# ay-lab/fithic

Measured on AMD Instinct MI355X. Metric: contact-pairs/sec through spline+p-value+BH pass (5 kb cis, whole node), higher is better.
Workload: dtype f64

## Files before the change

fithic_amd/csrc/fhx_bdtrc.hpp:

```cpp
#pragma once
#include <hip/hip_runtime.h>
#include <cstdint>

namespace fhx {
namespace dev {

constexpr double kMachEp = 1.11022302462515654042E-16;
constexpr double kMaxLog = 7.09782712893383996732E2;
constexpr double kMinLog = -7.451332191019412076235E2;
constexpr double kMaxGam = 171.624376956302725;
constexpr double kBig = 4.503599627370496e15;
constexpr double kBigInv = 2.22044604925031308085e-16;

struct BinomTables {
    const double* lbeta;
    const double* inv_beta;
    double n;
    int small_n;
};

__device__ __forceinline__ double cephes_log1p(double x) {
    double z = 1.0 + x;
    if (z < 0.70710678118654752440 || z > 1.41421356237309504880) return log(z);
    z = x * x;
// ... 551 lines not shown
    if (p < 0.0 || p > 1.0 || T.n < fk) return __builtin_nan("");
    if (fk < 0) return 1.0;
    if (fk == T.n) return 0.0;
    const double dn = T.n - fk;
    if (count == 1) {
        if (p < 0.01) return -cephes_expm1(dn * cephes_log1p(-p));
        return 1.0 - pow(1.0 - p, dn);
    }
    return incbet(fk + 1.0, dn, p, T.lbeta[count], T.small_n ? T.inv_beta[count] : 0.0);
}

__device__ __forceinline__ double bdtrc_count_trivial(int count, const BinomTables& T, double p) {
    if (isnan(p)) return p;
    const double fk = (double)count - 1.0;
    if (p < 0.0 || p > 1.0 || T.n < fk) return __builtin_nan("");
    if (fk < 0) return 1.0;
    if (fk == T.n) return 0.0;
    const double dn = T.n - fk;
    if (count == 1) {
        if (p < 0.01) return -cephes_expm1(dn * cephes_log1p(-p));
        return 1.0 - pow(1.0 - p, dn);
    }
    return p <= 0.0 ? 0.0 : 1.0;
}

__device__ __forceinline__ bool bdtrc_is_closed_form(int count, double n_total, double p) {
    return count == 1 && p >= 0.0 && p <= 1.0 && n_total > 0.0;
}
__device__ __forceinline__ double bdtrc_closed_form(double n_total, double p) {
    if (p < 0.01) return -cephes_expm1(n_total * cephes_log1p(-p));
    return 1.0 - pow(1.0 - p, n_total);
}

__device__ __forceinline__ double bdtrc_count_trivial_open(int count, const BinomTables& T, double p) {
    if (isnan(p)) return p;
    const double fk = (double)count - 1.0;
    if (p < 0.0 || p > 1.0 || T.n < fk) return __builtin_nan("");
    if (fk < 0) return 1.0;
    if (fk == T.n) return 0.0;
    return p <= 0.0 ? 0.0 : 1.0;
}

__device__ __forceinline__ int bdtrc_class(int count, double n_total, double p) {
    if (isnan(p)) return BC_TRIVIAL;
    const double fk = (double)count - 1.0;
    if (p < 0.0 || p > 1.0 || n_total < fk || fk < 0 || fk == n_total || count == 1) return BC_TRIVIAL;
    const double aa = fk + 1.0, bb = n_total - fk, xx = p;
    if (xx <= 0.0 || xx >= 1.0) return BC_TRIVIAL;
    if (bb * xx <= 1.0 && xx <= 0.95) return BC_PSERIES;
    const double w = 1.0 - xx;
    double a, b, x;
    bool swapped;
    if (xx > aa / (aa + bb)) {
        swapped = true; a = bb; b = aa; x = w;
        if (b * x <= 1.0 && x <= 0.95) return BC_PSERIES;
    } else {
        swapped = false; a = aa; b = bb; x = xx;
    }
    const double y = x * (a + b - 2.0) - (a - 1.0);
    if (y < 0.0) return swapped ? BC_CF_SWAPPED : BC_CF_BCF;
    return BC_CF_BD;
}

struct ClsRow {
    double tA, tB, tC, tD, tE, pad0, pad1, pad2;
};

__device__ __forceinline__ bool cls_pred(int which, double aa, double bb, double xx) {
    const double w = 1.0 - xx;
    switch (which) {
        case 0: return bb * xx <= 1.0 && xx <= 0.95;
        case 2: return aa * w <= 1.0 && w <= 0.95;
// ... 116 lines not shown
```

fithic_amd/csrc/fhx_ctx.hpp:

```cpp
#pragma once
#include <hip/hip_runtime.h>

#include <atomic>
#include <functional>
#include <chrono>
#include <thread>
#include <memory>
#include <sys/stat.h>
#include <unistd.h>
#include <deque>
#include <mutex>
#include <map>
#include <condition_variable>
#include <algorithm>
#include <climits>
#include <cstddef>
#include <cmath>
#include <cstdio>
#include <cstdlib>
#include <cstring>
#include <string>
#include <vector>

#include "../../include/fithic_mi355x.h"
// ... 61 lines not shown
    int n_table;
    double min_x, max_x;
    long long dist_low, dist_up;
    double total_intra, total_inter;
};

constexpr int K2_THREADS = 256;

constexpr int K2_QUEUES = dev::BC_COUNT - 1;

struct QEntry {
    unsigned int row;
    int count;
    double prior;
};

constexpr int K2_MAX_SHARDS = 2048;

struct QSpan {
    QEntry* base;
    long long cap_s;
    int dir;
    int n_shards;
    const unsigned long long* count;
};
__device__ __forceinline__ QEntry* qentry(const QSpan& q, int shard, long long j) {
    return q.base + (long long)shard * q.cap_s + (long long)q.dir * j;
}

struct K2Queues {
    QSpan q[K2_QUEUES + 1];
    unsigned long long* count;
    unsigned int* heavy_hist;
};

constexpr int K2H_BUCKETS = 2048;
constexpr int K2H_BLOCKS = 1024;
__device__ __forceinline__ int k2h_bucket(int signed_count);

struct CutoffToHost {
    volatile unsigned long long* words = nullptr;
    unsigned long long ticket = 0;
    unsigned int* done = nullptr;
    unsigned long long* zero_me = nullptr;
};

constexpr int K3_DENSE_PERCENT = 35;
constexpr int K2_COUNTER_WORDS = 8;
constexpr int FDR_BUCKETS = 51;

struct DeviceWords {
    unsigned long long bh_kept;
    unsigned long long bh_cutoff;
    unsigned long long bh_below;
    unsigned long long array_kept;
    unsigned long long array_cutoff;
    unsigned long long sort_n;
    unsigned long long run_total;
    unsigned long long nf_keys;
    unsigned long long outliers_added;
    unsigned long long first_dup;
    unsigned long long memo_overflow;
    alignas(128) unsigned long long k2_redo;
    unsigned long long k2_next[K2_COUNTER_WORDS - 1];
    alignas(128) unsigned long long k3_dense;
    unsigned long long k3_sparse;
// ... 343 lines not shown
    DeviceScratch() = default;
    explicit DeviceScratch(ScratchPool* p) : pool(p) {}
    ~DeviceScratch() {
        for (auto& b : v) {
            if (pool)
                pool->give(b.first, b.second);
            else
                (void)hipFree(b.first);
        }
    }
    template <typename T>
    hipError_t get(T** p, size_t bytes) {
        bytes = std::max<size_t>(bytes, 16);
        if (pool) {
            size_t real = 0;
            if (void* q = pool->take(bytes, &real)) {
                *p = (T*)q;
                v.emplace_back(q, real);
                return hipSuccess;
            }
        }
        const hipError_t e = hipMalloc((void**)p, bytes);
        if (e == hipSuccess) v.emplace_back((void*)*p, bytes);
        return e;
    }
};

inline int grid_for(int64_t n, int threads, int max_blocks = 256 * 8) {
    const int64_t b = (n + threads - 1) / threads;
    return (int)std::max<int64_t>(1, std::min<int64_t>(b, max_blocks));
}

inline int k2_classify_grid(int64_t n) {
    return grid_for(n, K2_CL_TILE, K2_MAX_SHARDS);
}
inline long long k2_shard_capacity(int64_t n) {
    const long long tiles = std::max<long long>(1, (n + K2_CL_TILE - 1) / K2_CL_TILE), grid = k2_classify_grid(n);
    return ((tiles + grid - 1) / grid) * (long long)K2_CL_TILE;
}


int build_slot_tables(fhx_ctx* ctx);
int run_ids(fhx_ctx* ctx, const unsigned long long* keys, int64_t n, unsigned int* ids, unsigned int* tile_scratch, int64_t* n_runs);
int alloc_row_arrays(fhx_ctx* ctx, int64_t n, int64_t n_dist);
int ingest_device_rows_nonfixed(fhx_ctx* ctx, const int32_t* c1, const int32_t* m1, const int32_t* c2, const int32_t* m2,
                                const int32_t* cnt, int64_t n);
int ingest_device_rows(fhx_ctx* ctx, const int32_t* c1, const int32_t* m1, const int32_t* c2, const int32_t* m2, const int32_t* cnt,
                       int64_t n);
int pass_stats_nonfixed(fhx_ctx* ctx, fhx_stats* out);
int launch_k1(fhx_ctx* ctx);
void fold_kernel_events(fhx_ctx* ctx);
void before_rerecord(fhx_ctx* ctx, int group);
K2Params make_k2_params(fhx_ctx* c);
void launch_k2_extras(fhx_ctx* ctx, const K2Params& P, int64_t n_rows, double* d_expcc, double* d_b1, double* d_b2);
int ensure_sort_scratch(fhx_ctx* ctx);
int sort_blocks_for(int64_t n_hint);
int radix_sort_pairs(fhx_ctx* ctx, unsigned long long* keys[2], unsigned int* vals[2], const unsigned long long* counter, int passes,
                     int* result_buf, int64_t n_hint = -1);
void launch_rs_scan(fhx_ctx* ctx, int nblk);
int fill_top_hist(fhx_ctx* ctx);
void launch_k3_cutoff(fhx_ctx* ctx, const unsigned long long* hist, double n_tests, unsigned long long* d_cutoff,
                      unsigned long long* n_below, unsigned long long dense_min, unsigned long long* dense_flag, const CutoffToHost& host,
                      unsigned long long sparse_max = 0, unsigned long long* sparse_flag = nullptr);
void launch_bh_tile_max(fhx_ctx* ctx, int tiles, const unsigned long long* keys, const unsigned long long* n_ptr, int64_t n_fixed,
                        double n_tests, double rank0, double* tile_max);
void launch_bh_scan_tiles(fhx_ctx* ctx, double* tile_max, const unsigned long long* n_ptr, int64_t n_fixed, double carry_in,
// ... 10 lines not shown
```

fithic_amd/csrc/fhx_k2.hip:

```cpp
#include "fhx_ctx.hpp"

namespace fhx {

__device__ __forceinline__ double prior_by_search(const K2Params& P, long long dist) {
    double look = (double)dist;
    if (look < P.min_x) look = P.min_x;
    if (look > P.max_x) look = P.max_x;
    int lo = 0, hi = P.n_table;
    while (lo < hi) {
        const int mid = (lo + hi) >> 1;
        if (P.table_x[mid] < look)
            lo = mid + 1;
        else
            hi = mid;
    }
    return P.table_y[min(lo, P.n_table - 1)];
}

template <int NF = -1>
__device__ __forceinline__ bool row_prior(const K2Params& P, int l1, int l2, double& prior, bool& is_inter) {
    const bool inter = l2 < 0;
    const int s2 = inter ? ~l2 : l2;
    const double b1 = P.no_bias ? 1.0 : P.slot_bias[l1], b2 = P.no_bias ? 1.0 : P.slot_bias[s2];
    if ((b1 < 0 || b2 < 0) && !inter) return false;
    if (!inter && P.mode != FHX_MODE_INTER_ONLY) {
        if (NF == 1 || (NF == -1 && P.nonfixed)) {
            const long long dist = llabs((long long)P.slot_mid[l1] - (long long)P.slot_mid[s2]);
            if (dist < P.dist_low || dist > P.dist_up) return false;
            prior = prior_by_search(P, dist) * (b1 * b2);
            is_inter = false;
            return true;
        }
        const int d = abs(l1 - s2);
        if (d < P.lo_idx || d > P.hi_idx) return false;
        prior = P.prior_lut[d] * (b1 * b2);
        is_inter = false;
        return true;
    }
    if (P.mode == FHX_MODE_INTRA_ONLY) return false;
    prior = P.inter_chr_prob * (b1 * b2);
    is_inter = true;
    return true;
}

template <int ITEMS>
__device__ __forceinline__ void rows_prior_fixed(const K2Params& P, const int (&l1)[ITEMS], const int (&l2)[ITEMS], double (&prior)[ITEMS],
                                                 bool (&is_inter)[ITEMS], bool (&live)[ITEMS]) {
    double b1[ITEMS], b2[ITEMS], tab[ITEMS];
    int dist[ITEMS];
#pragma unroll
    for (int r = 0; r < ITEMS; ++r) {
        const bool inter = l2[r] < 0;
        const int s2 = inter ? ~l2[r] : l2[r];
        dist[r] = abs(l1[r] - s2);
        b1[r] = P.no_bias ? 1.0 : P.slot_bias[l1[r]];
        b2[r] = P.no_bias ? 1.0 : P.slot_bias[s2];
        tab[r] = P.prior_lut[min(dist[r], P.lut_len - 1)];
    }
#pragma unroll
    for (int r = 0; r < ITEMS; ++r) {
        const bool inter = l2[r] < 0;
        const double bb = b1[r] * b2[r];
        const bool as_intra = !inter && P.mode != FHX_MODE_INTER_ONLY;
        const bool discarded = (b1[r] < 0 || b2[r] < 0) && !inter;
        const bool in_range = dist[r] >= P.lo_idx && dist[r] <= P.hi_idx;
        live[r] = !discarded && (as_intra ? in_range : P.mode != FHX_MODE_INTRA_ONLY);
        is_inter[r] = !as_intra;
        prior[r] = live[r] ? (as_intra ? tab[r] : P.inter_chr_prob) * bb : 1.0;
    }
}

constexpr int K2_HIST_BINS = 4096;
struct FusedHist {
    unsigned int* h;
    unsigned int ones;
    bool on;
    __device__ __forceinline__ void init(unsigned int* lds, const unsigned long long* global) {
        h = lds;
        ones = 0;
        on = global != nullptr;
        if (on) {
            for (int i = threadIdx.x; i < K2_HIST_BINS; i += blockDim.x) h[i] = 0;
            __syncthreads();
        }
    }
    __device__ __forceinline__ void add(double v) {
        if (!on) return;
        if (v == 1.0)
            ++ones;
        else if (v == v) {
            unsigned long long bits = (unsigned long long)__double_as_longlong(v);
            if (bits == 0x8000000000000000ull) bits = 0ull;
            atomicAdd(&h[min((unsigned int)(bits >> 50), (unsigned int)K2_HIST_BINS - 1u)], 1u);
        }
    }
    __device__ __forceinline__ void add_wave_min(double v, bool valid) {
        if (!on) return;
        valid = valid && v == v;
        unsigned long long key = valid ? (unsigned long long)__double_as_longlong(v) : ~0ull;
        if (key == 0x8000000000000000ull) key = 0ull;
#pragma unroll
        for (int s = 32; s >= 1; s >>= 1) {
            const unsigned long long o = __shfl_xor(key, s, 64);
            key = o < key ? o : key;
        }
        const unsigned int n = (unsigned int)__popcll(__ballot(valid));
        if ((threadIdx.x & 63) == 0 && n) atomicAdd(&h[min((unsigned int)(key >> 50), (unsigned int)K2_HIST_BINS - 1u)], n);
    }
    __device__ __forceinline__ void flush(unsigned long long* global) {
        if (!on) return;
        const unsigned int w = (unsigned int)wave_sum_i64((long long)ones);
        if ((threadIdx.x & 63) == 0 && w) atomicAdd(&h[0x3FF0000000000000ull >> 50], w);
        __syncthreads();
        for (int i = threadIdx.x; i < K2_HIST_BINS; i += blockDim.x)
            if (h[i]) atomicAdd(&global[i], (unsigned long long)h[i]);
    }
};

template <bool SCATTERED>
__device__ __forceinline__ void store_p(double* dst, double v) {
    if (SCATTERED)
        __builtin_nontemporal_store(v, dst);
    else
        *dst = v;
}

constexpr int K2_TB_COUNTS = 128;
template <int NF, int WPE, int TABLE, bool HOIST = false, bool PACK = false>
__global__ __launch_bounds__(K2_THREADS) __attribute__((amdgpu_waves_per_eu(WPE, WPE))) void k2_classify(K2Params P, K2Queues Q) {
    static_assert(!HOIST || NF == 0, "the hoisted gathers are the fixed-size path's");
    static_assert(TABLE == 0 || TABLE == 3, "table variants 1 and 2 were measured and dropped");
    constexpr int ITEMS = K2_CL_ITEMS, WAVES = K2_THREADS / 64, WAVE_ROWS = 64 * ITEMS;
    __shared__ unsigned int cnt[K2_QUEUES + 1];
    __shared__ double cf_prior[WAVES][WAVE_ROWS];
    __shared__ unsigned short cf_idx[WAVES][WAVE_ROWS];
    __shared__ unsigned int hist_lds[K2_HIST_BINS];
    __shared__ unsigned int heavy_lds[K2H_BUCKETS];
    __shared__ double tb_lds[TABLE == 3 ? 2 * K2_TB_COUNTS : 1];
    if (TABLE == 3) {
        static_assert(2 * K2_TB_COUNTS <= K2_THREADS, "one thread per table entry");
        if (threadIdx.x < 2 * K2_TB_COUNTS) {
            const int c = threadIdx.x & (K2_TB_COUNTS - 1);
            const double n_total = threadIdx.x < K2_TB_COUNTS ? P.intra.n : P.inter.n;
            const double fk = (double)c - 1.0;
            const double aa = fk + 1.0, bb = n_total - fk;
            tb_lds[threadIdx.x] = aa / (aa + bb);
        }
    }
    if (threadIdx.x <= K2_QUEUES) cnt[threadIdx.x] = 0;
    const bool count_heavy = Q.heavy_hist != nullptr;
    if (count_heavy)
        for (int d = threadIdx.x; d < K2H_BUCKETS; d += K2_THREADS) heavy_lds[d] = 0;
    FusedHist H;
    H.init(hist_lds, P.top_hist);
    __syncthreads();
    const int lane = threadIdx.x & 63;
    const int wave = threadIdx.x >> 6;
    const unsigned long long lane_lt = (1ull << lane) - 1ull;
    const int shard = (int)blockIdx.x;
    const int64_t tiles = (P.n + K2_CL_TILE - 1) / K2_CL_TILE;
    const int4* a4 = reinterpret_cast<const int4*>(P.loc1);
    const int4* b4 = reinterpret_cast<const int4*>(P.loc2);
    const int4* c4 = reinterpret_cast<const int4*>(P.count);
    for (int64_t t = blockIdx.x; t < tiles; t += gridDim.x) {
        const int64_t wave_row0 = t * K2_CL_TILE + (int64_t)wave * WAVE_ROWS;
        const int64_t row0 = wave_row0 + lane * ITEMS;
        int l1_of[ITEMS] = {0, 0, 0, 0}, l2_of[ITEMS] = {0, 0, 0, 0}, count_of[ITEMS] = {0, 0, 0, 0};
        if (row0 < P.n) {
            const int4 a = a4[row0 >> 2], b = b4[row0 >> 2], c = c4[row0 >> 2];
            l1_of[0] = a.x; l1_of[1] = a.y; l1_of[2] = a.z; l1_of[3] = a.w;
            l2_of[0] = b.x; l2_of[1] = b.y; l2_of[2] = b.z; l2_of[3] = b.w;
            count_of[0] = c.x; count_of[1] = c.y; count_of[2] = c.z; count_of[3] = c.w;
            if (HOIST && row0 + ITEMS > P.n) {
#pragma unroll
                for (int r = 1; r < ITEMS; ++r)
                    if (row0 + r >= P.n) l1_of[r] = l2_of[r] = 0;
            }
        }
        int cls_of[ITEMS];
        double prior_of[ITEMS];
        bool inter_of[ITEMS], live_of[ITEMS];
        if (HOIST) rows_prior_fixed<ITEMS>(P, l1_of, l2_of, prior_of, inter_of, live_of);
#pragma unroll
        for (int r = 0; r < ITEMS; ++r) {
            const int64_t i = row0 + r;
            int cls = -1;
            double prior = 1.0;
            int c = count_of[r];
            if (i < P.n) {
                double pv = 1.0;
                bool is_inter = false;
                cls = 0;
                bool live;
                if (HOIST) {
                    live = live_of[r];
                    prior = prior_of[r];
                    is_inter = inter_of[r];
                } else {
                    live = row_prior<NF>(P, l1_of[r], l2_of[r], prior, is_inter);
                }
                if (live) {
                    const dev::BinomTables& T = is_inter ? P.inter : P.intra;
                    if (TABLE == 3) {
                        double tB;
                        if (c >= 0 && c < K2_TB_COUNTS) {
                            tB = tb_lds[(is_inter ? K2_TB_COUNTS : 0) + c];
                        } else {
                            const double fk = (double)c - 1.0;
                            const double aa = fk + 1.0, bb = T.n - fk;
                            tB = aa / (aa + bb);
                        }
                        cls = dev::bdtrc_class_tb(c, T.n, prior, tB);
                    } else {
                        cls = dev::bdtrc_class(c, T.n, prior);
                    }
                    if (cls == dev::BC_TRIVIAL) {
                        if (dev::bdtrc_is_closed_form(c, T.n, prior))
                            cls = prior < 0.01 ? K2_CLOSED_LOCAL : K2_CLOSED;
                        else
                            pv = dev::bdtrc_count_trivial_open(c, T, prior);
                    }
                    if (is_inter) c = -c;
                }
                if (cls == 0) {
                    P.p[i] = pv;
                    H.add(pv);
                }
            }
            cls_of[r] = cls;
            count_of[r] = c;
            prior_of[r] = prior;
        }
        unsigned int before_cls[ITEMS];
        unsigned int tot[K2_CLASSES] = {0u, 0u, 0u, 0u, 0u, 0u};
        static_assert(K2_CLASSES == 6 && K2_QUEUES == 4, "lane k reserves class k; the sixth class is wave-local");
        if (PACK) {
            unsigned int mine[2] = {0u, 0u};
            unsigned int shift_of[ITEMS];
#pragma unroll
            for (int r = 0; r < ITEMS; ++r) {
                const int k = cls_of[r] - 1;
                const int f = k >= 3 ? k - 3 : k;
                shift_of[r] = 10u * (unsigned int)(f < 0 ? 0 : f);
                const unsigned int one = k >= 0 ? (1u << shift_of[r]) : 0u;
                mine[0] += k < 3 ? one : 0u;
                mine[1] += k >= 3 ? one : 0u;
            }
            const unsigned int incl0 = wave_incl_sum_u32(mine[0]), incl1 = wave_incl_sum_u32(mine[1]);
            const unsigned int all0 = (unsigned int)__builtin_amdgcn_readlane((int)incl0, 63), all1 = (unsigned int)__builtin_amdgcn_readlane((int)incl1, 63);
            tot[0] = all0 & 1023u; tot[1] = (all0 >> 10) & 1023u; tot[2] = (all0 >> 20) & 1023u;
            tot[3] = all1 & 1023u; tot[4] = (all1 >> 10) & 1023u; tot[5] = (all1 >> 20) & 1023u;
            unsigned int run[2] = {incl0 - mine[0], incl1 - mine[1]};
#pragma unroll
            for (int r = 0; r < ITEMS; ++r) {
                const int k = cls_of[r] - 1;
                const unsigned int word = k >= 3 ? run[1] : run[0];
                before_cls[r] = (word >> shift_of[r]) & 1023u;
                const unsigned int one = k >= 0 ? (1u << shift_of[r]) : 0u;
                run[0] += k < 3 ? one : 0u;
                run[1] += k >= 3 ? one : 0u;
            }
        } else {
#pragma unroll
            for (int r = 0; r < ITEMS; ++r) {
                before_cls[r] = 0;
#pragma unroll
                for (int k = 1; k <= K2_CLASSES; ++k) {
                    const unsigned long long m = __ballot(cls_of[r] == k);
                    if (cls_of[r] == k) before_cls[r] = tot[k - 1] + (unsigned int)__popcll(m & lane_lt);
                    tot[k - 1] += (unsigned int)__popcll(m);
                }
            }
        }
        const unsigned int my_tot = lane == 0 ? tot[0] : (lane == 1 ? tot[1] : (lane == 2 ? tot[2] : (lane == 3 ? tot[3] : tot[4])));
        unsigned int my_base = 0;
        if (lane <= K2_QUEUES && my_tot) my_base = atomicAdd(&cnt[lane], my_tot);
        unsigned int wave_base[K2_QUEUES + 1];
#pragma unroll
        for (int k = 0; k <= K2_QUEUES; ++k) wave_base[k] = __shfl(my_base, k, 64);
#pragma unroll
        for (int r = 0; r < ITEMS; ++r) {
            const int k = cls_of[r] - 1;
            if (k >= 0 && k <= K2_QUEUES) {
                const unsigned int wb = k == 0 ? wave_base[0] : (k == 1 ? wave_base[1] : (k == 2 ? wave_base[2] : (k == 3 ? wave_base[3] : wave_base[4])));
                QEntry e;
                e.row = (unsigned int)(row0 + r);
                e.count = count_of[r];
                e.prior = prior_of[r];
                *qentry(Q.q[k], shard, (long long)(wb + before_cls[r])) = e;
                if (k == dev::BC_CF_SWAPPED - 1 && count_heavy) atomicAdd(&heavy_lds[k2h_bucket(e.count)], 1u);
            } else if (cls_of[r] == K2_CLOSED_LOCAL) {
                cf_prior[wave][before_cls[r]] = prior_of[r];
                cf_idx[wave][before_cls[r]] = (unsigned short)((lane * ITEMS + r) | (count_of[r] < 0 ? 0x8000 : 0));
            }
        }
        __builtin_amdgcn_fence(__ATOMIC_RELEASE, "wavefront");
        __builtin_amdgcn_wave_barrier();
        __builtin_amdgcn_fence(__ATOMIC_ACQUIRE, "wavefront");
        const unsigned int n_local = tot[K2_CLASSES - 1];
        for (unsigned int j = lane; j < n_local; j += 64) {
            const unsigned int ix = cf_idx[wave][j];
            const double n_total = (ix & 0x8000u) ? P.inter.n : P.intra.n;
            const double pr = cf_prior[wave][j];
            const double pv = -dev::cephes_expm1(n_total * dev::cephes_log1p(-pr));
            P.p[wave_row0 + (ix & 0x7FFFu)] = pv;
            H.add(pv);
        }
        __builtin_amdgcn_fence(__ATOMIC_RELEASE, "wavefront");
        __builtin_amdgcn_wave_barrier();
    }
    __syncthreads();
    if (threadIdx.x <= K2_QUEUES) Q.count[(size_t)threadIdx.x * K2_MAX_SHARDS + shard] = cnt[threadIdx.x];
    if (count_heavy)
        for (int d = threadIdx.x; d < K2H_BUCKETS; d += K2_THREADS)
            if (heavy_lds[d]) atomicAdd(&Q.heavy_hist[(size_t)d * K2H_BLOCKS + (shard & (K2H_BLOCKS - 1))], heavy_lds[d]);
    H.flush(P.top_hist);
}

__global__ __launch_bounds__(K2_THREADS) void k2_closed(K2Params P, QSpan q, unsigned long long* __restrict__ zero_words,
                                                        unsigned long long* __restrict__ cutoff_word) {
    __shared__ unsigned int hist_lds[K2_HIST_BINS];
    if (blockIdx.x == 0 && threadIdx.x < K2_COUNTER_WORDS) zero_words[threadIdx.x] = 0ull;
    if (blockIdx.x == 0 && threadIdx.x == K2_COUNTER_WORDS) *cutoff_word = KEY_KEEP_ALL;
    FusedHist H;
    H.init(hist_lds, P.top_hist);
    for (int sh = blockIdx.x; sh < q.n_shards; sh += gridDim.x) {
        const long long n = (long long)q.count[sh];
        for (long long j = threadIdx.x; j < n; j += blockDim.x) {
            const QEntry e = *qentry(q, sh, j);
            const double pv = dev::bdtrc_closed_form(e.count < 0 ? P.inter.n : P.intra.n, e.prior);
            store_p<false>(P.p + e.row, pv);
            H.add(pv);
        }
    }
    H.flush(P.top_hist);
}

struct QDense {
    static constexpr int PAIRS = K2_MAX_SHARDS / 2;
    unsigned int* prefix;
    const unsigned long long* count;
    __device__ __forceinline__ void build(const QSpan& q, unsigned int* prefix_lds, unsigned int* wave_tot) {
        static_assert(PAIRS % K2_THREADS == 0, "whole pairs per thread");
        constexpr int PER = PAIRS / K2_THREADS;
        prefix = prefix_lds;
        count = q.count;
        unsigned int c[PER], s = 0;
#pragma unroll
// ... 628 lines not shown
    if (Q->heavy_hist && !prezeroed)
        FHX_HIP(hipMemsetAsync(ctx->d_block_hist, 0, (size_t)K2H_BUCKETS * K2H_BLOCKS * sizeof(unsigned int), ctx->stream));
    ctx->k2_shards = plan.n_shards;
    auto span = [&](int cls, QEntry* buf, int dir) {
        Q->q[cls - 1] = QSpan{dir > 0 ? buf : buf + plan.cap_s - 1, plan.cap_s, dir, plan.n_shards, Q->count + (size_t)(cls - 1) * K2_MAX_SHARDS};
    };
    span(dev::BC_CF_SWAPPED, ctx->d_queue[0], 1);
    span(dev::BC_PSERIES, ctx->d_queue[0], -1);
    span(dev::BC_CF_BCF, ctx->d_queue[1], 1);
    span(dev::BC_CF_BD, ctx->d_queue[1], -1);
    span(K2_CLOSED, ctx->d_queue_sorted, 1);
    return FHX_OK;
}

template <int CLS, bool SMALL_N>
static void launch_k2_queue(fhx_ctx* ctx, const K2Params& P, const K2Queues& Q) {
    hipLaunchKernelGGL(HIP_KERNEL_NAME(k2_queue<CLS, SMALL_N>), dim3(2 * resident_grid(ctx, k2_queue<CLS, SMALL_N>)), dim3(K2_THREADS), 0,
                       ctx->stream, P, Q.q[CLS - 1]);
}
template <int CLS, bool SMALL_N>
static void launch_k2_queue_by_count(fhx_ctx* ctx, const K2Params& P, const K2Queues& Q) {
    constexpr int PIECE = SMALL_N ? 4 : 5;
    hipLaunchKernelGGL(HIP_KERNEL_NAME(k2_queue_by_count<CLS, SMALL_N, PIECE>), dim3(resident_grid(ctx, k2_queue_by_count<CLS, SMALL_N, PIECE>)),
                       dim3(K2_THREADS), 0, ctx->stream, P, Q.q[CLS - 1], (unsigned int*)(ctx->d_words->k2_next + CLS));
}
template <int ROWS, int WAVES, bool SMALL_N>
static void launch_k2h_heavy(fhx_ctx* ctx, const K2Params& P, QEntry* redo) {
    hipLaunchKernelGGL(HIP_KERNEL_NAME(k2h_heavy<ROWS, WAVES, SMALL_N>), dim3(256 * WAVES), dim3(K2H_THREADS), 0, ctx->stream,
                       K2HeavyParams{P.intra, P.inter, P.p, P.top_hist}, (const QEntry*)ctx->d_queue_sorted, (const unsigned int*)ctx->d_k2h_off,
                       (const unsigned int*)ctx->d_digit_total, (const dev::CfRow*)ctx->d_cf_tab, redo, &ctx->d_words->k2_redo,
                       (unsigned int*)ctx->d_words->k2_next);
}

template <bool SMALL_N>
static int launch_k2(fhx_ctx* ctx, const K2Plan& plan, const K2Params& P, const K2Queues& Q) {
    const dim3 cgrid(plan.n_shards), block(K2_THREADS);
    if (P.nonfixed)
        hipLaunchKernelGGL(HIP_KERNEL_NAME(k2_classify<1, 4, 0>), cgrid, block, 0, ctx->stream, P, Q);
    else
        hipLaunchKernelGGL(HIP_KERNEL_NAME(k2_classify<0, 4, 3, true, true>), cgrid, block, 0, ctx->stream, P, Q);
    hipLaunchKernelGGL(k2_closed, dim3(256 * 8), block, 0, ctx->stream, P, Q.q[K2_CLOSED - 1], &ctx->d_words->k2_redo, &ctx->d_words->bh_cutoff);
    if (plan.legacy_heavy) {
        FHX_HIP(hipEventRecord(ctx->ev[6], ctx->stream));
        launch_k2_queue<dev::BC_CF_SWAPPED, SMALL_N>(ctx, P, Q);
        FHX_HIP(hipEventRecord(ctx->ev[7], ctx->stream));
        ctx->ev_folded[3] = false;
        launch_k2_queue_by_count<dev::BC_CF_BD, SMALL_N>(ctx, P, Q);
        launch_k2_queue_by_count<dev::BC_CF_BCF, SMALL_N>(ctx, P, Q);
        launch_k2_queue<dev::BC_PSERIES, SMALL_N>(ctx, P, Q);
        return FHX_OK;
    }
    static_assert(K2H_BUCKETS == RADIX && K2H_BLOCKS == SORT_BLOCKS, "the radix sort's count matrix and scan are reused");
    QEntry* hq = ctx->d_queue[0];
    launch_rs_scan(ctx, (int)SORT_BLOCKS);
    hipLaunchKernelGGL(k2h_offsets_and_tables, dim3(K2H_GENERIC + 1), dim3(1024), 0, ctx->stream, (const unsigned int*)ctx->d_digit_total,
                       ctx->d_k2h_off, 64u * (unsigned int)plan.heavy_rows, P.intra.n, P.inter.n, ctx->d_cf_tab);
    hipLaunchKernelGGL(k2h_scatter, dim3(K2H_BLOCKS), dim3(K2H_THREADS), 0, ctx->stream, Q.q[dev::BC_CF_SWAPPED - 1],
                       (const unsigned int*)ctx->d_block_hist, (const unsigned int*)ctx->d_k2h_off, ctx->d_queue_sorted);
    launch_k2_queue<dev::BC_PSERIES, SMALL_N>(ctx, P, Q);
    FHX_HIP(hipEventRecord(ctx->ev[6], ctx->stream));
    if (plan.heavy_rows == 2) launch_k2h_heavy<2, 8, SMALL_N>(ctx, P, hq);
    else launch_k2h_heavy<4, 4, SMALL_N>(ctx, P, hq);
    FHX_HIP(hipEventRecord(ctx->ev[7], ctx->stream));
    ctx->ev_folded[3] = false;
    hipLaunchKernelGGL(k2h_generic, dim3(256 * 4), dim3(K2_THREADS), 0, ctx->stream, P, (const QEntry*)ctx->d_queue_sorted,
                       (const unsigned int*)ctx->d_k2h_off, (const unsigned int*)ctx->d_digit_total, (const QEntry*)hq,
                       (const unsigned long long*)&ctx->d_words->k2_redo);
    launch_k2_queue_by_count<dev::BC_CF_BD, SMALL_N>(ctx, P, Q);
    launch_k2_queue_by_count<dev::BC_CF_BCF, SMALL_N>(ctx, P, Q);
    return FHX_OK;
}

static int k2_fused_hist(fhx_ctx* ctx, bool prezeroed, K2Params* P) {
// ... 480 lines not shown
```

Before: 14.17 billion.

## Slim k2_classify kernel arguments and specialize on no_bias

Replaces the large K2Params/K2Queues kernel arguments of the classify kernel with a compact dedicated parameter struct that flattens queue bases, directions and mode flags. It adds a compile-time no_bias specialization and computes per-wave queue pointers once through LDS instead of shuffling bases. It also restructures the per-row loop so that dead rows are written up front and the packed prefix-count path is always used. The aim is to cut scalar argument loads, VALU work and register pressure in the classify pass, at the cost of more template variants and an added env override for grid size.

```diff
diff --git a/fithic_amd/csrc/fhx_bdtrc.hpp b/fithic_amd/csrc/fhx_bdtrc.hpp
--- a/fithic_amd/csrc/fhx_bdtrc.hpp
+++ b/fithic_amd/csrc/fhx_bdtrc.hpp
@@ -607,12 +607,12 @@
     return 1.0 - pow(1.0 - p, n_total);
 }
 
-__device__ __forceinline__ double bdtrc_count_trivial_open(int count, const BinomTables& T, double p) {
+__device__ __forceinline__ double bdtrc_count_trivial_open(int count, double n_total, double p) {
     if (isnan(p)) return p;
     const double fk = (double)count - 1.0;
-    if (p < 0.0 || p > 1.0 || T.n < fk) return __builtin_nan("");
+    if (p < 0.0 || p > 1.0 || n_total < fk) return __builtin_nan("");
     if (fk < 0) return 1.0;
-    if (fk == T.n) return 0.0;
+    if (fk == n_total) return 0.0;
     return p <= 0.0 ? 0.0 : 1.0;
 }
 
diff --git a/fithic_amd/csrc/fhx_ctx.hpp b/fithic_amd/csrc/fhx_ctx.hpp
--- a/fithic_amd/csrc/fhx_ctx.hpp
+++ b/fithic_amd/csrc/fhx_ctx.hpp
@@ -117,6 +117,33 @@
     QSpan q[K2_QUEUES + 1];
     unsigned long long* count;
     unsigned int* heavy_hist;
+};
+
+struct K2ClassifyParams {
+    const int32_t *loc1, *loc2, *count;
+    const double* slot_bias;
+    const double* prior_lut;
+    double* p;
+    unsigned long long* top_hist;
+    QEntry* q_base[K2_QUEUES + 1];
+    unsigned long long* q_count;
+    unsigned int* heavy_hist;
+    long long cap_s;
+    int64_t n;
+    double n_intra, n_inter;
+    double inter_chr_prob;
+    int lut_len, lo_idx, hi_idx;
+    unsigned int q_down;
+    bool intra_by_distance;
+    bool other_rows_live;
+};
+struct K2ClassifyParamsNF : K2ClassifyParams {
+    const int32_t* slot_mid;
+    const double *table_x, *table_y;
+    int n_table, mode;
+    double min_x, max_x;
+    long long dist_low, dist_up;
+    bool no_bias;
 };
 
 constexpr int K2H_BUCKETS = 2048;
@@ -526,6 +553,10 @@
 }
 
 inline int k2_classify_grid(int64_t n) {
+    if (const char* e = std::getenv("FHX_K2_CLASSIFY_GRID")) {
+        const long long g = std::atoll(e);
+        if (g >= 1) return (int)std::min<long long>(g, K2_MAX_SHARDS);
+    }
     return grid_for(n, K2_CL_TILE, K2_MAX_SHARDS);
 }
 inline long long k2_shard_capacity(int64_t n) {
diff --git a/fithic_amd/csrc/fhx_k2.hip b/fithic_amd/csrc/fhx_k2.hip
--- a/fithic_amd/csrc/fhx_k2.hip
+++ b/fithic_amd/csrc/fhx_k2.hip
@@ -2,7 +2,8 @@
 
 namespace fhx {
 
-__device__ __forceinline__ double prior_by_search(const K2Params& P, long long dist) {
+template <class PT>
+__device__ __forceinline__ double prior_by_search(const PT& P, long long dist) {
     double look = (double)dist;
     if (look < P.min_x) look = P.min_x;
     if (look > P.max_x) look = P.max_x;
@@ -17,14 +18,16 @@
     return P.table_y[min(lo, P.n_table - 1)];
 }
 
-template <int NF = -1>
-__device__ __forceinline__ bool row_prior(const K2Params& P, int l1, int l2, double& prior, bool& is_inter) {
+template <int NF = -1, class PT = K2Params>
+__device__ __forceinline__ bool row_prior(const PT& P, int l1, int l2, double& prior, bool& is_inter) {
     const bool inter = l2 < 0;
     const int s2 = inter ? ~l2 : l2;
     const double b1 = P.no_bias ? 1.0 : P.slot_bias[l1], b2 = P.no_bias ? 1.0 : P.slot_bias[s2];
     if ((b1 < 0 || b2 < 0) && !inter) return false;
     if (!inter && P.mode != FHX_MODE_INTER_ONLY) {
-        if (NF == 1 || (NF == -1 && P.nonfixed)) {
+        bool by_search = NF == 1;
+        if constexpr (NF == -1) by_search = P.nonfixed;
+        if (by_search) {
             const long long dist = llabs((long long)P.slot_mid[l1] - (long long)P.slot_mid[s2]);
             if (dist < P.dist_low || dist > P.dist_up) return false;
             prior = prior_by_search(P, dist) * (b1 * b2);
@@ -43,9 +46,9 @@
     return true;
 }
 
-template <int ITEMS>
-__device__ __forceinline__ void rows_prior_fixed(const K2Params& P, const int (&l1)[ITEMS], const int (&l2)[ITEMS], double (&prior)[ITEMS],
-                                                 bool (&is_inter)[ITEMS], bool (&live)[ITEMS]) {
+template <int ITEMS, bool NO_BIAS>
+__device__ __forceinline__ void rows_prior_fixed(const K2ClassifyParams& P, const int (&l1)[ITEMS], const int (&l2)[ITEMS],
+                                                 double (&prior)[ITEMS], bool (&is_inter)[ITEMS], bool (&live)[ITEMS]) {
     double b1[ITEMS], b2[ITEMS], tab[ITEMS];
     int dist[ITEMS];
 #pragma unroll
@@ -53,18 +56,18 @@
         const bool inter = l2[r] < 0;
         const int s2 = inter ? ~l2[r] : l2[r];
         dist[r] = abs(l1[r] - s2);
-        b1[r] = P.no_bias ? 1.0 : P.slot_bias[l1[r]];
-        b2[r] = P.no_bias ? 1.0 : P.slot_bias[s2];
+        b1[r] = NO_BIAS ? 1.0 : P.slot_bias[l1[r]];
+        b2[r] = NO_BIAS ? 1.0 : P.slot_bias[s2];
         tab[r] = P.prior_lut[min(dist[r], P.lut_len - 1)];
     }
 #pragma unroll
     for (int r = 0; r < ITEMS; ++r) {
         const bool inter = l2[r] < 0;
         const double bb = b1[r] * b2[r];
-        const bool as_intra = !inter && P.mode != FHX_MODE_INTER_ONLY;
+        const bool as_intra = !inter && P.intra_by_distance;
         const bool discarded = (b1[r] < 0 || b2[r] < 0) && !inter;
         const bool in_range = dist[r] >= P.lo_idx && dist[r] <= P.hi_idx;
-        live[r] = !discarded && (as_intra ? in_range : P.mode != FHX_MODE_INTRA_ONLY);
+        live[r] = live[r] && !discarded && (as_intra ? in_range : P.other_rows_live);
         is_inter[r] = !as_intra;
         prior[r] = live[r] ? (as_intra ? tab[r] : P.inter_chr_prob) * bb : 1.0;
     }
@@ -126,29 +129,36 @@
 }
 
 constexpr int K2_TB_COUNTS = 128;
-template <int NF, int WPE, int TABLE, bool HOIST = false, bool PACK = false>
-__global__ __launch_bounds__(K2_THREADS) __attribute__((amdgpu_waves_per_eu(WPE, WPE))) void k2_classify(K2Params P, K2Queues Q) {
-    static_assert(!HOIST || NF == 0, "the hoisted gathers are the fixed-size path's");
-    static_assert(TABLE == 0 || TABLE == 3, "table variants 1 and 2 were measured and dropped");
+template <int NF>
+struct K2ClassifyArgs {
+    using type = K2ClassifyParams;
+};
+template <>
+struct K2ClassifyArgs<1> {
+    using type = K2ClassifyParamsNF;
+};
+template <int NF, bool NO_BIAS>
+__global__ __launch_bounds__(K2_THREADS) __attribute__((amdgpu_waves_per_eu(4, 4))) void k2_classify(const typename K2ClassifyArgs<NF>::type P) {
+    static_assert(NF == 0 || NF == 1, "fixed-size loci or arbitrary ones");
+    static_assert(NF == 0 || !NO_BIAS, "k2_classify<1> reads no_bias at run time (row_prior<1>)");
     constexpr int ITEMS = K2_CL_ITEMS, WAVES = K2_THREADS / 64, WAVE_ROWS = 64 * ITEMS;
     __shared__ unsigned int cnt[K2_QUEUES + 1];
+    __shared__ QEntry* wave_q[WAVES][8];
     __shared__ double cf_prior[WAVES][WAVE_ROWS];
     __shared__ unsigned short cf_idx[WAVES][WAVE_ROWS];
     __shared__ unsigned int hist_lds[K2_HIST_BINS];
     __shared__ unsigned int heavy_lds[K2H_BUCKETS];
-    __shared__ double tb_lds[TABLE == 3 ? 2 * K2_TB_COUNTS : 1];
-    if (TABLE == 3) {
-        static_assert(2 * K2_TB_COUNTS <= K2_THREADS, "one thread per table entry");
-        if (threadIdx.x < 2 * K2_TB_COUNTS) {
-            const int c = threadIdx.x & (K2_TB_COUNTS - 1);
-            const double n_total = threadIdx.x < K2_TB_COUNTS ? P.intra.n : P.inter.n;
-            const double fk = (double)c - 1.0;
-            const double aa = fk + 1.0, bb = n_total - fk;
-            tb_lds[threadIdx.x] = aa / (aa + bb);
-        }
+    __shared__ double tb_lds[2 * K2_TB_COUNTS];
+    static_assert(2 * K2_TB_COUNTS <= K2_THREADS, "one thread per table entry");
+    if (threadIdx.x < 2 * K2_TB_COUNTS) {
+        const int c = threadIdx.x & (K2_TB_COUNTS - 1);
+        const double n_total = threadIdx.x < K2_TB_COUNTS ? P.n_intra : P.n_inter;
+        const double fk = (double)c - 1.0;
+        const double aa = fk + 1.0, bb = n_total - fk;
+        tb_lds[threadIdx.x] = aa / (aa + bb);
     }
     if (threadIdx.x <= K2_QUEUES) cnt[threadIdx.x] = 0;
-    const bool count_heavy = Q.heavy_hist != nullptr;
+    const bool count_heavy = P.heavy_hist != nullptr;
     if (count_heavy)
         for (int d = threadIdx.x; d < K2H_BUCKETS; d += K2_THREADS) heavy_lds[d] = 0;
     FusedHist H;
@@ -156,8 +166,19 @@
     __syncthreads();
     const int lane = threadIdx.x & 63;
     const int wave = threadIdx.x >> 6;
-    const unsigned long long lane_lt = (1ull << lane) - 1ull;
     const int shard = (int)blockIdx.x;
+    static_assert(K2_QUEUES + 1 == 5, "five queues: lanes 0..4");
+    QEntry* my_q = nullptr;
+    {
+        const long long region = (long long)shard * P.cap_s;
+        QEntry* const q0 = P.q_base[0];
+        QEntry* const q1 = P.q_base[1];
+        QEntry* const q2 = P.q_base[2];
+        QEntry* const q3 = P.q_base[3];
+        QEntry* const q4 = P.q_base[4];
+        my_q = (lane == 0 ? q0 : (lane == 1 ? q1 : (lane == 2 ? q2 : (lane == 3 ? q3 : q4)))) + region;
+    }
+    const bool my_down = ((P.q_down >> (lane & 7)) & 1u) != 0u;
     const int64_t tiles = (P.n + K2_CL_TILE - 1) / K2_CL_TILE;
     const int4* a4 = reinterpret_cast<const int4*>(P.loc1);
     const int4* b4 = reinterpret_cast<const int4*>(P.loc2);
@@ -165,142 +186,128 @@
     for (int64_t t = blockIdx.x; t < tiles; t += gridDim.x) {
         const int64_t wave_row0 = t * K2_CL_TILE + (int64_t)wave * WAVE_ROWS;
         const int64_t row0 = wave_row0 + lane * ITEMS;
+        const int64_t left = P.n - row0;
+        const int n_here = left >= ITEMS ? ITEMS : (left > 0 ? (int)left : 0);
         int l1_of[ITEMS] = {0, 0, 0, 0}, l2_of[ITEMS] = {0, 0, 0, 0}, count_of[ITEMS] = {0, 0, 0, 0};
-        if (row0 < P.n) {
+        if (n_here > 0) {
             const int4 a = a4[row0 >> 2], b = b4[row0 >> 2], c = c4[row0 >> 2];
             l1_of[0] = a.x; l1_of[1] = a.y; l1_of[2] = a.z; l1_of[3] = a.w;
             l2_of[0] = b.x; l2_of[1] = b.y; l2_of[2] = b.z; l2_of[3] = b.w;
             count_of[0] = c.x; count_of[1] = c.y; count_of[2] = c.z; count_of[3] = c.w;
-            if (HOIST && row0 + ITEMS > P.n) {
+            if (NF == 0 && n_here < ITEMS) {
 #pragma unroll
                 for (int r = 1; r < ITEMS; ++r)
-                    if (row0 + r >= P.n) l1_of[r] = l2_of[r] = 0;
+                    if (r >= n_here) l1_of[r] = l2_of[r] = 0;
             }
         }
-        int cls_of[ITEMS];
         double prior_of[ITEMS];
         bool inter_of[ITEMS], live_of[ITEMS];
-        if (HOIST) rows_prior_fixed<ITEMS>(P, l1_of, l2_of, prior_of, inter_of, live_of);
+#pragma unroll
+        for (int r = 0; r < ITEMS; ++r) live_of[r] = r < n_here;
+        if constexpr (NF == 0) {
+            rows_prior_fixed<ITEMS, NO_BIAS>(P, l1_of, l2_of, prior_of, inter_of, live_of);
+        } else {
+#pragma unroll
+            for (int r = 0; r < ITEMS; ++r) {
+                prior_of[r] = 1.0;
+                inter_of[r] = false;
+                if (live_of[r]) live_of[r] = row_prior<NF>(P, l1_of[r], l2_of[r], prior_of[r], inter_of[r]);
+            }
+        }
+        double* const p_lane = P.p + row0;
 #pragma unroll
         for (int r = 0; r < ITEMS; ++r) {
-            const int64_t i = row0 + r;
+            if (r < n_here && !live_of[r]) {
+                p_lane[r] = 1.0;
+                ++H.ones;
+            }
+        }
+        int cls_of[ITEMS];
+#pragma unroll
+        for (int r = 0; r < ITEMS; ++r) {
             int cls = -1;
-            double prior = 1.0;
-            int c = count_of[r];
-            if (i < P.n) {
-                double pv = 1.0;
-                bool is_inter = false;
-                cls = 0;
-                bool live;
-                if (HOIST) {
-                    live = live_of[r];
-                    prior = prior_of[r];
-                    is_inter = inter_of[r];
+            if (live_of[r]) {
+                const int c = count_of[r];
+                const double n_total = inter_of[r] ? P.n_inter : P.n_intra;
+                double tB;
+                if (c >= 0 && c < K2_TB_COUNTS) {
+                    tB = tb_lds[(inter_of[r] ? K2_TB_COUNTS : 0) + c];
                 } else {
-                    live = row_prior<NF>(P, l1_of[r], l2_of[r], prior, is_inter);
+                    const double fk = (double)c - 1.0;
+                    const double aa = fk + 1.0, bb = n_total - fk;
+                    tB = aa / (aa + bb);
                 }
-                if (live) {
-                    const dev::BinomTables& T = is_inter ? P.inter : P.intra;
-                    if (TABLE == 3) {
-                        double tB;
-                        if (c >= 0 && c < K2_TB_COUNTS) {
-                            tB = tb_lds[(is_inter ? K2_TB_COUNTS : 0) + c];
-                        } else {
-                            const double fk = (double)c - 1.0;
-                            const double aa = fk + 1.0, bb = T.n - fk;
-                            tB = aa / (aa + bb);
-                        }
-                        cls = dev::bdtrc_class_tb(c, T.n, prior, tB);
+                cls = dev::bdtrc_class_tb(c, n_total, prior_of[r], tB);
+                if (cls == dev::BC_TRIVIAL) {
+                    if (dev::bdtrc_is_closed_form(c, n_total, prior_of[r])) {
+                        cls = prior_of[r] < 0.01 ? K2_CLOSED_LOCAL : K2_CLOSED;
                     } else {
-                        cls = dev::bdtrc_class(c, T.n, prior);
+                        const double pv = dev::bdtrc_count_trivial_open(c, n_total, prior_of[r]);
+                        p_lane[r] = pv;
+                        H.add(pv);
+                        cls = -1;
                     }
-                    if (cls == dev::BC_TRIVIAL) {
-                        if (dev::bdtrc_is_closed_form(c, T.n, prior))
-                            cls = prior < 0.01 ? K2_CLOSED_LOCAL : K2_CLOSED;
-                        else
-                            pv = dev::bdtrc_count_trivial_open(c, T, prior);
-                    }
-                    if (is_inter) c = -c;
-                }
-                if (cls == 0) {
-                    P.p[i] = pv;
-                    H.add(pv);
                 }
             }
             cls_of[r] = cls;
-            count_of[r] = c;
-            prior_of[r] = prior;
         }
         unsigned int before_cls[ITEMS];
-        unsigned int tot[K2_CLASSES] = {0u, 0u, 0u, 0u, 0u, 0u};
         static_assert(K2_CLASSES == 6 && K2_QUEUES == 4, "lane k reserves class k; the sixth class is wave-local");
-        if (PACK) {
-            unsigned int mine[2] = {0u, 0u};
-            unsigned int shift_of[ITEMS];
-#pragma unroll
-            for (int r = 0; r < ITEMS; ++r) {
-                const int k = cls_of[r] - 1;
-                const int f = k >= 3 ? k - 3 : k;
-                shift_of[r] = 10u * (unsigned int)(f < 0 ? 0 : f);
-                const unsigned int one = k >= 0 ? (1u << shift_of[r]) : 0u;
-                mine[0] += k < 3 ? one : 0u;
-                mine[1] += k >= 3 ? one : 0u;
-            }
-            const unsigned int incl0 = wave_incl_sum_u32(mine[0]), incl1 = wave_incl_sum_u32(mine[1]);
-            const unsigned int all0 = (unsigned int)__builtin_amdgcn_readlane((int)incl0, 63), all1 = (unsigned int)__builtin_amdgcn_readlane((int)incl1, 63);
-            tot[0] = all0 & 1023u; tot[1] = (all0 >> 10) & 1023u; tot[2] = (all0 >> 20) & 1023u;
-            tot[3] = all1 & 1023u; tot[4] = (all1 >> 10) & 1023u; tot[5] = (all1 >> 20) & 1023u;
-            unsigned int run[2] = {incl0 - mine[0], incl1 - mine[1]};
-#pragma unroll
-            for (int r = 0; r < ITEMS; ++r) {
-                const int k = cls_of[r] - 1;
-                const unsigned int word = k >= 3 ? run[1] : run[0];
-                before_cls[r] = (word >> shift_of[r]) & 1023u;
-                const unsigned int one = k >= 0 ? (1u << shift_of[r]) : 0u;
-                run[0] += k < 3 ? one : 0u;
-                run[1] += k >= 3 ? one : 0u;
-            }
-        } else {
-#pragma unroll
-            for (int r = 0; r < ITEMS; ++r) {
-                before_cls[r] = 0;
-#pragma unroll
-                for (int k = 1; k <= K2_CLASSES; ++k) {
-                    const unsigned long long m = __ballot(cls_of[r] == k);
-                    if (cls_of[r] == k) before_cls[r] = tot[k - 1] + (unsigned int)__popcll(m & lane_lt);
-                    tot[k - 1] += (unsigned int)__popcll(m);
-                }
-            }
-        }
-        const unsigned int my_tot = lane == 0 ? tot[0] : (lane == 1 ? tot[1] : (lane == 2 ? tot[2] : (lane == 3 ? tot[3] : tot[4])));
-        unsigned int my_base = 0;
-        if (lane <= K2_QUEUES && my_tot) my_base = atomicAdd(&cnt[lane], my_tot);
-        unsigned int wave_base[K2_QUEUES + 1];
-#pragma unroll
-        for (int k = 0; k <= K2_QUEUES; ++k) wave_base[k] = __shfl(my_base, k, 64);
+        unsigned int mine[2] = {0u, 0u};
+        unsigned int shift_of[ITEMS];
+#pragma unroll
+        for (int r = 0; r < ITEMS; ++r) {
+            const int k = cls_of[r] - 1;
+            const int f = k >= 3 ? k - 3 : k;
+            shift_of[r] = 10u * (unsigned int)(f < 0 ? 0 : f);
+            const unsigned int one = k >= 0 ? (1u << shift_of[r]) : 0u;
+            mine[0] += k < 3 ? one : 0u;
+            mine[1] += k >= 3 ? one : 0u;
+        }
+        const unsigned int incl0 = wave_incl_sum_u32(mine[0]), incl1 = wave_incl_sum_u32(mine[1]);
+        const unsigned int all0 = (unsigned int)__builtin_amdgcn_readlane((int)incl0, 63), all1 = (unsigned int)__builtin_amdgcn_readlane((int)incl1, 63);
+        unsigned int run[2] = {incl0 - mine[0], incl1 - mine[1]};
+#pragma unroll
+        for (int r = 0; r < ITEMS; ++r) {
+            const int k = cls_of[r] - 1;
+            const unsigned int word = k >= 3 ? run[1] : run[0];
+            before_cls[r] = (word >> shift_of[r]) & 1023u;
+            const unsigned int one = k >= 0 ? (1u << shift_of[r]) : 0u;
+            run[0] += k < 3 ? one : 0u;
+            run[1] += k >= 3 ? one : 0u;
+        }
+        const unsigned int my_tot = lane == 0 ? (all0 & 1023u) : (lane == 1 ? ((all0 >> 10) & 1023u) : (lane == 2 ? ((all0 >> 20) & 1023u)
+                                    : (lane == 3 ? (all1 & 1023u) : ((all1 >> 10) & 1023u))));
+        if (lane <= K2_QUEUES) {
+            const unsigned int my_base = my_tot ? atomicAdd(&cnt[lane], my_tot) : 0u;
+            wave_q[wave][lane] = my_down ? my_q - my_base : my_q + my_base;
+        }
+        __builtin_amdgcn_fence(__ATOMIC_RELEASE, "wavefront");
+        __builtin_amdgcn_wave_barrier();
+        __builtin_amdgcn_fence(__ATOMIC_ACQUIRE, "wavefront");
 #pragma unroll
         for (int r = 0; r < ITEMS; ++r) {
             const int k = cls_of[r] - 1;
             if (k >= 0 && k <= K2_QUEUES) {
-                const unsigned int wb = k == 0 ? wave_base[0] : (k == 1 ? wave_base[1] : (k == 2 ? wave_base[2] : (k == 3 ? wave_base[3] : wave_base[4])));
                 QEntry e;
                 e.row = (unsigned int)(row0 + r);
-                e.count = count_of[r];
+                e.count = inter_of[r] ? -count_of[r] : count_of[r];
                 e.prior = prior_of[r];
-                *qentry(Q.q[k], shard, (long long)(wb + before_cls[r])) = e;
+                QEntry* const first = wave_q[wave][k];
+                *(((P.q_down >> k) & 1u) ? first - before_cls[r] : first + before_cls[r]) = e;
                 if (k == dev::BC_CF_SWAPPED - 1 && count_heavy) atomicAdd(&heavy_lds[k2h_bucket(e.count)], 1u);
             } else if (cls_of[r] == K2_CLOSED_LOCAL) {
                 cf_prior[wave][before_cls[r]] = prior_of[r];
-                cf_idx[wave][before_cls[r]] = (unsigned short)((lane * ITEMS + r) | (count_of[r] < 0 ? 0x8000 : 0));
+                cf_idx[wave][before_cls[r]] = (unsigned short)((lane * ITEMS + r) | (inter_of[r] ? 0x8000 : 0));
             }
         }
         __builtin_amdgcn_fence(__ATOMIC_RELEASE, "wavefront");
         __builtin_amdgcn_wave_barrier();
         __builtin_amdgcn_fence(__ATOMIC_ACQUIRE, "wavefront");
-        const unsigned int n_local = tot[K2_CLASSES - 1];
+        const unsigned int n_local = (all1 >> 20) & 1023u;
         for (unsigned int j = lane; j < n_local; j += 64) {
             const unsigned int ix = cf_idx[wave][j];
-            const double n_total = (ix & 0x8000u) ? P.inter.n : P.intra.n;
+            const double n_total = (ix & 0x8000u) ? P.n_inter : P.n_intra;
             const double pr = cf_prior[wave][j];
             const double pv = -dev::cephes_expm1(n_total * dev::cephes_log1p(-pr));
             P.p[wave_row0 + (ix & 0x7FFFu)] = pv;
@@ -310,10 +317,10 @@
         __builtin_amdgcn_wave_barrier();
     }
     __syncthreads();
-    if (threadIdx.x <= K2_QUEUES) Q.count[(size_t)threadIdx.x * K2_MAX_SHARDS + shard] = cnt[threadIdx.x];
+    if (threadIdx.x <= K2_QUEUES) P.q_count[(size_t)threadIdx.x * K2_MAX_SHARDS + shard] = cnt[threadIdx.x];
     if (count_heavy)
         for (int d = threadIdx.x; d < K2H_BUCKETS; d += K2_THREADS)
-            if (heavy_lds[d]) atomicAdd(&Q.heavy_hist[(size_t)d * K2H_BLOCKS + (shard & (K2H_BLOCKS - 1))], heavy_lds[d]);
+            if (heavy_lds[d]) atomicAdd(&P.heavy_hist[(size_t)d * K2H_BLOCKS + (shard & (K2H_BLOCKS - 1))], heavy_lds[d]);
     H.flush(P.top_hist);
 }
 
@@ -1008,13 +1015,54 @@
                        (unsigned int*)ctx->d_words->k2_next);
 }
 
+static K2ClassifyParamsNF classify_params(const K2Params& P, const K2Queues& Q) {
+    K2ClassifyParamsNF C{};
+    C.loc1 = P.loc1;
+    C.loc2 = P.loc2;
+    C.count = P.count;
+    C.slot_bias = P.slot_bias;
+    C.prior_lut = P.prior_lut;
+    C.p = P.p;
+    C.top_hist = P.top_hist;
+    for (int k = 0; k <= K2_QUEUES; ++k) {
+        C.q_base[k] = Q.q[k].base;
+        if (Q.q[k].dir < 0) C.q_down |= 1u << k;
+    }
+    C.q_count = Q.count;
+    C.heavy_hist = Q.heavy_hist;
+    C.cap_s = Q.q[0].cap_s;
+    C.n = P.n;
+    C.n_intra = P.intra.n;
+    C.n_inter = P.inter.n;
+    C.inter_chr_prob = P.inter_chr_prob;
+    C.lut_len = P.lut_len;
+    C.lo_idx = P.lo_idx;
+    C.hi_idx = P.hi_idx;
+    C.intra_by_distance = P.mode != FHX_MODE_INTER_ONLY;
+    C.other_rows_live = P.mode != FHX_MODE_INTRA_ONLY;
+    C.slot_mid = P.slot_mid;
+    C.table_x = P.table_x;
+    C.table_y = P.table_y;
+    C.n_table = P.n_table;
+    C.mode = P.mode;
+    C.min_x = P.min_x;
+    C.max_x = P.max_x;
+    C.dist_low = P.dist_low;
+    C.dist_up = P.dist_up;
+    C.no_bias = P.no_bias;
+    return C;
+}
+
 template <bool SMALL_N>
 static int launch_k2(fhx_ctx* ctx, const K2Plan& plan, const K2Params& P, const K2Queues& Q) {
     const dim3 cgrid(plan.n_shards), block(K2_THREADS);
+    const K2ClassifyParamsNF C = classify_params(P, Q);
     if (P.nonfixed)
-        hipLaunchKernelGGL(HIP_KERNEL_NAME(k2_classify<1, 4, 0>), cgrid, block, 0, ctx->stream, P, Q);
+        hipLaunchKernelGGL(HIP_KERNEL_NAME(k2_classify<1, false>), cgrid, block, 0, ctx->stream, C);
+    else if (P.no_bias)
+        hipLaunchKernelGGL(HIP_KERNEL_NAME(k2_classify<0, true>), cgrid, block, 0, ctx->stream, (const K2ClassifyParams&)C);
     else
-        hipLaunchKernelGGL(HIP_KERNEL_NAME(k2_classify<0, 4, 3, true, true>), cgrid, block, 0, ctx->stream, P, Q);
+        hipLaunchKernelGGL(HIP_KERNEL_NAME(k2_classify<0, false>), cgrid, block, 0, ctx->stream, (const K2ClassifyParams&)C);
     hipLaunchKernelGGL(k2_closed, dim3(256 * 8), block, 0, ctx->stream, P, Q.q[K2_CLOSED - 1], &ctx->d_words->k2_redo, &ctx->d_words->bh_cutoff);
     if (plan.legacy_heavy) {
         FHX_HIP(hipEventRecord(ctx->ev[6], ctx->stream));
diff --git a/profiles/isa_counts.py b/profiles/isa_counts.py
--- /dev/null
+++ b/profiles/isa_counts.py
@@ -0,0 +1,54 @@
+#!/usr/bin/env python3
+import collections
+import os
+import re
+import subprocess
+import sys
+import tempfile
+
+LLVM = os.environ.get("LLVM_BIN", "/opt/rocm/llvm/bin")
+
+
+def main():
+    obj, pattern = sys.argv[1], sys.argv[2]
+    with tempfile.TemporaryDirectory() as tmp:
+        co = os.path.join(tmp, "device.co")
+        fat = os.path.join(tmp, "fatbin")
+        subprocess.check_call([os.path.join(LLVM, "llvm-objcopy"), "--dump-section", ".hip_fatbin=" + fat, obj, os.path.join(tmp, "rest.o")])
+        subprocess.check_call([os.path.join(LLVM, "clang-offload-bundler"), "--type=o", "--unbundle", "--input=" + fat, "--output=" + co,
+                               "--targets=hipv4-amdgcn-amd-amdhsa--gfx950"])
+        dis = subprocess.run([os.path.join(LLVM, "llvm-objdump"), "-d", "--no-show-raw-insn", co], capture_output=True, text=True, check=True).stdout
+        notes = subprocess.run([os.path.join(LLVM, "llvm-readelf"), "--notes", co], capture_output=True, text=True, check=True).stdout
+    demangle = lambda names: subprocess.run(["c++filt"] + names, capture_output=True, text=True, check=True).stdout.split("\n")
+    meta = {}
+    for block in notes.split("- .agpr_count:")[1:]:
+        get = lambda key: (re.search(r"\.%s:\s*(\S+)" % key, block) or [None, "?"])[1]
+        meta[get("name")] = (get("vgpr_count"), get("sgpr_count"), get("group_segment_fixed_size"), get("vgpr_spill_count"), get("sgpr_spill_count"))
+    counts, cur = {}, None
+    for line in dis.split("\n"):
+        m = re.match(r"^[0-9a-f]+ <(\S+)>:", line)
+        if m:
+            cur = counts.setdefault(m.group(1), collections.Counter())
+            continue
+        t = line.strip().split()
+        if cur is None or not t or not re.match(r"^[a-z]", t[0]):
+            continue
+        op = t[0]
+        cur["VALU" if op.startswith("v_") else "SALU" if op.startswith("s_") else "other"] += 1
+        for key in ("s_cbranch_execz", "s_and_saveexec", "v_readlane", "v_writelane", "v_mad_u64_u32", "v_mov_b32", "v_cndmask_b32", "v_div_scale_f64"):
+            if op.startswith(key):
+                cur[key] += 1
+    names = [n for n in counts if n in meta]
+    for name, nice in zip(names, demangle(names)):
+        if pattern not in nice:
+            continue
+        c, (vgpr, sgpr, lds, vspill, sspill) = counts[name], meta[name]
+        print(nice)
+        print("  VALU %d  SALU %d  s_cbranch_execz %d  s_and_saveexec %d  v_readlane %d  v_writelane %d  v_mad_u64_u32 %d  v_mov_b32 %d  "
+              "v_cndmask_b32 %d  v_div_scale_f64 %d" % (c["VALU"], c["SALU"], c["s_cbranch_execz"], c["s_and_saveexec"], c["v_readlane"], c["v_writelane"],
+                                                       c["v_mad_u64_u32"], c["v_mov_b32"], c["v_cndmask_b32"], c["v_div_scale_f64"]))
+        print("  VGPRs %s  SGPRs %s  LDS %s bytes  spilled VGPRs %s  spilled SGPRs %s" % (vgpr, sgpr, lds, vspill, sspill))
+
+
+if __name__ == "__main__":
+    main()
```

After: 14.29 billion, median of 6. No clear change (+0.8%).
